# chengzhag/PanFusion

Hardware: AMD Instinct MI355X
Metric: DDIM denoise steps/sec, 512x1024 pano + 20x512^2 views (higher is better)
Workload: dtype fp16; 1 GPU; cfg2: 512x1024 pano + 20x512^2 views, CFG pair, SD-2-base UNet shapes; views=20, cfg_pair=True, hip_graphs=True, parallelism=single

## Files before the change

### include/panfusion_hip.h

```cpp
#ifndef PANFUSION_HIP_H
#define PANFUSION_HIP_H

#include <stddef.h>
#include <stdint.h>

#ifdef __cplusplus
extern "C" {
#endif

typedef enum { PF_OK = 0, PF_ERR_ARG = 1, PF_ERR_LAUNCH = 2, PF_ERR_UNSUPPORTED = 3 } pf_status;
typedef enum { PF_BF16 = 0, PF_F16 = 1, PF_F32 = 2, PF_U8 = 3, PF_F64 = 4 } pf_dtype;

int pf_version(void);
const char* pf_last_error_string(void);


pf_status pf_e2p_grid(const double* host_fov, const double* host_theta, const double* host_phi,
                      int ncam, int eh, int ew, int h, int w,
                      float* map_x, float* map_y, float* lonlat, void* stream);

pf_status pf_p2e_grid(const double* host_fov, const double* host_theta, const double* host_phi,
                      int ncam, int ph, int pw, int h, int w,
                      float* map_u, float* map_v, uint8_t* mask, void* stream);

// ... 164 lines not shown
    int h_out, w_out;
    int ksize;
    int stride;
    int pad;
    int upsample;
    const void* w;
    int n_out;
    const float* bias;
    const float* rowvec;
    int rowvec_ld;
    const void* residual;
    int res_ld;
    int res_dtype;
    void* out;
    int out_ld;
    int out_dtype;
    int dtype;
    int batch;
    long a_bstride, w_bstride, out_bstride, res_bstride;
    int epilogue;
    void* workspace;
    size_t workspace_bytes;
    float* gn_partial;
    int wrap_pad;
    int crop;
    int* tickets;
    int n_tickets;
    int split3;
    int subpixel;
    int gn_rows;
    int a_src_dtype;
    const float* a_scale;
    const float* a_shift;
} pf_conv_desc;

enum { PF_EPILOGUE_NONE = 0, PF_EPILOGUE_GEGLU = 1, PF_EPILOGUE_SPLIT = 2 };

size_t pf_conv_gemm_workspace_size(const pf_conv_desc* desc);
int pf_conv_gemm_gn_rows(const pf_conv_desc* desc);
int pf_conv_gemm_kernel_id(const pf_conv_desc* desc);
typedef struct {
    int kernel;
    int mrep, nrep;
    int block_rows;
    int waves;
    int ring_slots;
    int splits;
    int kb_per_split;
    int m_split;
    int tail_splits, tail_kb;
    int gn_rows;
    int n_tickets;
    size_t workspace_bytes;
} pf_conv_plan;
pf_status pf_conv_gemm_plan(const pf_conv_desc* desc, int want_moments, pf_conv_plan* out);
pf_status pf_debug_gemm_profile(void* device_buffer, long capacity_blocks);
pf_status pf_conv_gemm(const pf_conv_desc* desc, void* stream);

typedef struct {
    const void* a; int a_ld;
    const void* w;
    const float* bias;
    const float* residual; int res_ld;
    void* out; int out_ld;
    void* out_vt; int vt_ld; int rows_per_batch; long vt_bs;
    const float* ln_gamma; const float* ln_beta; float ln_eps; void* ln_out; int ln_ld;
// ... 179 lines not shown
```

### panfusion_amd/_lib.py

```python
import ctypes as C
import os

_HERE = os.path.dirname(os.path.abspath(__file__))
LIB_PATH = os.environ.get("PF_HIP_LIB") or os.path.join(_HERE, "libpanfusion_hip.so")

PF_OK = 0
PF_BF16, PF_F16, PF_F32, PF_U8, PF_F64 = 0, 1, 2, 3, 4

c_void_p, c_int, c_long, c_float, c_size_t = C.c_void_p, C.c_int, C.c_long, C.c_float, C.c_size_t
c_dp = C.POINTER(C.c_double)


class ConvDesc(C.Structure):
    _fields_ = [
        ("a0", c_void_p), ("a1", c_void_p), ("c0", c_int), ("c1", c_int),
        ("a0_ld", c_int), ("a1_ld", c_int),
        ("n_img", c_int), ("h_in", c_int), ("w_in", c_int), ("h_out", c_int), ("w_out", c_int),
        ("ksize", c_int), ("stride", c_int), ("pad", c_int), ("upsample", c_int),
        ("w", c_void_p), ("n_out", c_int),
        ("bias", c_void_p), ("rowvec", c_void_p), ("rowvec_ld", c_int),
        ("residual", c_void_p), ("res_ld", c_int), ("res_dtype", c_int),
        ("out", c_void_p), ("out_ld", c_int), ("out_dtype", c_int), ("dtype", c_int),
        ("batch", c_int),
        ("a_bstride", c_long), ("w_bstride", c_long), ("out_bstride", c_long), ("res_bstride", c_long),
        ("epilogue", c_int), ("workspace", c_void_p), ("workspace_bytes", c_size_t),
        ("gn_partial", c_void_p), ("wrap_pad", c_int), ("crop", c_int),
        ("tickets", c_void_p), ("n_tickets", c_int), ("split3", c_int), ("subpixel", c_int), ("gn_rows", c_int),
        ("a_src_dtype", c_int), ("a_scale", c_void_p), ("a_shift", c_void_p),
    ]


class ConvPlan(C.Structure):
    _fields_ = [
        ("kernel", c_int), ("mrep", c_int), ("nrep", c_int), ("block_rows", c_int), ("waves", c_int), ("ring_slots", c_int),
        ("splits", c_int), ("kb_per_split", c_int), ("m_split", c_int), ("tail_splits", c_int), ("tail_kb", c_int),
        ("gn_rows", c_int), ("n_tickets", c_int), ("workspace_bytes", c_size_t),
    ]


class AttnDesc(C.Structure):
    _fields_ = [
        ("q", c_void_p), ("k", c_void_p), ("vt", c_void_p), ("out", c_void_p),
        ("dtype", c_int), ("B", c_int), ("H", c_int), ("D", c_int), ("nq", c_int), ("nk", c_int),
        ("q_ld", c_int), ("k_ld", c_int), ("vt_ld", c_int), ("o_ld", c_int),
        ("q_bs", c_long), ("k_bs", c_long), ("vt_bs", c_long), ("o_bs", c_long),
        ("scale", c_float),
        ("bias", c_void_p), ("bias_ld", c_long), ("flags", c_void_p), ("flags_ld", c_int),
        ("lse", c_void_p),
        ("workspace", c_void_p), ("workspace_bytes", c_size_t),
    ]


class AttnPlan(C.Structure):
    _fields_ = [
        ("kernel", c_int), ("pipelined", c_int), ("occupancy", c_int), ("msum", c_int), ("block_queries", c_int), ("threads", c_int),
        ("splits", c_int), ("split_tiles", c_int), ("grid_x", C.c_uint), ("grid_y", C.c_uint), ("grid_z", C.c_uint),
        ("workspace_bytes", c_size_t),
    ]


class LinearWsDesc(C.Structure):
# ... 252 lines not shown
```

### panfusion_amd/csrc/pf_gemm.hip

```cpp
#include "pf_common.h"
#include "pf_gemm_params.h"
#include "pf_gemm_walk.h"
#include <stdlib.h>
#include <algorithm>
#include <atomic>
#include <type_traits>

namespace pf {


template <typename T> struct Mfma;
template <> struct Mfma<Bf16> {
    typedef __attribute__((ext_vector_type(8))) __bf16 frag;
    static __device__ __forceinline__ f32x4 run(frag a, frag b, f32x4 c) {
        return __builtin_amdgcn_mfma_f32_16x16x32_bf16(a, b, c, 0, 0, 0);
    }
    static __device__ __forceinline__ void acc_agpr(frag a, frag b, f32x4& c) {
        asm volatile("v_mfma_f32_16x16x32_bf16 %0, %1, %2, %0" : "+a"(c) : "v"(a), "v"(b));
    }
};
template <> struct Mfma<F16> {
    typedef __attribute__((ext_vector_type(8))) _Float16 frag;
    static __device__ __forceinline__ f32x4 run(frag a, frag b, f32x4 c) {
        return __builtin_amdgcn_mfma_f32_16x16x32_f16(a, b, c, 0, 0, 0);
// ... 1324 lines not shown
    GemmParams p;
    params_from_desc(d, p);
    const pf_conv_plan g = plan_conv_gemm(p, batch, d->workspace != nullptr, d->gn_partial != nullptr);
    PF_REQUIRE(!(a32 && d->a_scale && g.kernel == 1 && g.block_rows == 256 && g.nrep == 5),
               "pf_conv_gemm: a_scale / a_shift are not available on the 256 x 160 tile of the 8-wave kernel (this problem's plan): use the pair form");
    PF_REQUIRE(!(a32 && d->a_scale) || (d->h_out * d->w_out) % 2 == 0, "pf_conv_gemm: a_scale needs an even number of rows per image");
    if (d->gn_partial) {
        PF_REQUIRE(g.gn_rows > 0, "pf_conv_gemm: gn_partial given but this problem cannot emit GroupNorm moments (ask pf_conv_gemm_gn_rows first)");
        PF_REQUIRE(aligned16(d->gn_partial), "pf_conv_gemm: gn_partial must be 16-byte aligned");
        PF_REQUIRE(d->gn_rows == g.gn_rows, "pf_conv_gemm: gn_partial is sized for runs of gn_rows = %d rows, but this launch's plan writes runs of %d rows (ask pf_conv_gemm_plan again)",
                   d->gn_rows, g.gn_rows);
        p.gn_partial = d->gn_partial;
        p.gn_rows = g.gn_rows;
    }
    {
        const long npix = static_cast<long>(d->n_img) * d->h_in * d->w_in;
        const long a0b = a32 ? ((npix - 1) * p.a0_ld + p.c0 / 2) * 4 : ((npix - 1) * p.a0_ld + p.c0) * 2;
        const long a1b = !p.a1 ? 0 : a32 ? ((npix - 1) * p.a1_ld + p.c1 / 2) * 4 : ((npix - 1) * p.a1_ld + p.c1) * 2;
        const long wb = static_cast<long>(p.N) * p.K * 2;
        PF_REQUIRE(a0b < (1L << 31) && a1b < (1L << 31) && wb < (1L << 31),
                   "pf_conv_gemm: each operand must be smaller than 2 GiB (32-bit buffer offsets)");
        p.a0_bytes = static_cast<unsigned>(a0b); p.a1_bytes = static_cast<unsigned>(a1b); p.w_bytes = static_cast<unsigned>(wb);
    }
    p.partial = static_cast<float*>(d->workspace);
    if (d->tickets && g.kernel != 2 && gemm_tuning().splitk_inkernel && d->workspace_bytes < (1ULL << 32)) {
        PF_REQUIRE(d->n_tickets >= g.n_tickets && (reinterpret_cast<uintptr_t>(d->tickets) & 3) == 0,
                   "pf_conv_gemm: %d arrival counters needed, %d given", g.n_tickets, d->n_tickets);
        p.tickets = d->tickets;
    }
    PF_REQUIRE(g.workspace_bytes == 0 || (d->workspace_bytes >= g.workspace_bytes && aligned16(d->workspace)),
               "pf_conv_gemm: workspace of %zu bytes (16-byte aligned) needed, got %zu", g.workspace_bytes, d->workspace_bytes);
    hipStream_t st = as_stream(stream);
    p.splits = g.splits; p.kb_per_split = g.kb_per_split;
    if (g.m_split == 0) return launch_pass(g, p, d->dtype, batch, st);
    GemmParams p2 = p;
    p.M = g.m_split;
    p2.m_begin = g.m_split; p2.splits = g.tail_splits; p2.kb_per_split = g.tail_kb;
    const pf_status s1 = launch_pass(g, p, d->dtype, batch, st);
    return s1 != PF_OK ? s1 : launch_pass(g, p2, d->dtype, batch, st);
}

extern "C" pf_status pf_debug_gemm_profile(void* device_buffer, long capacity_blocks) {
    const ProfState* s = device_buffer ? new ProfState{static_cast<unsigned long long*>(device_buffer), capacity_blocks} : nullptr;
    g_prof_state.store(s, std::memory_order_release);
    return PF_OK;
}
```

### panfusion_amd/csrc/pf_gemm_params.h

```cpp
#pragma once
#include <atomic>
#include <cstdlib>

#include "pf_common.h"

namespace pf {

struct GemmParams {
    const unsigned short* a0; const unsigned short* a1;
    int c0, c1, a0_ld, a1_ld;
    int h_in, w_in, h_out, w_out;
    int ksize, stride, pad, up;
    int wrap, crop;
    const unsigned short* w;
    int M, N, K;
    int m_begin;
    int rows_per_img;
    const float* bias; const float* rowvec; int rowvec_ld;
    const void* residual; int res_ld; int res_f32;
    void* out; int out_ld; int out_f32; int geglu;
    int split_out;
    long a_bs, w_bs, out_bs, res_bs;
    int mtiles, ntiles;
    int splits, kb_per_split;
    float* partial;
    int* tickets;
    int batch;
    unsigned a0_bytes, a1_bytes, w_bytes;
    int adv_img, adv_y, adv_x;
    unsigned long long* prof;
    int s3;
    float* gn_partial;
    int gn_rows;
    int fastseg;
    int a32;
    const float* a_scale; const float* a_shift;
    int subpix;
};

__device__ __forceinline__ void seg_pack(int& img_pix, int& y_msk, int x, int h_in, int w_in) {
    const int img = img_pix, y = y_msk;
    unsigned m = 0;
#pragma unroll
    for (int k = 0; k < 3; ++k) {
        m |= (static_cast<unsigned>(y + k) < static_cast<unsigned>(h_in) ? 1u : 0u) << k;
        m |= (static_cast<unsigned>(x + k) < static_cast<unsigned>(w_in) ? 16u : 0u) << k;
    }
    img_pix = static_cast<int>((static_cast<unsigned>(img) * static_cast<unsigned>(h_in) + static_cast<unsigned>(y)) * static_cast<unsigned>(w_in) + static_cast<unsigned>(x));
    y_msk = static_cast<int>(m);
}

__device__ __forceinline__ long out_row(const GemmParams& p, long bz, int m) {
    if (!p.subpix) return m;
    const int q = m / p.w_out, x = m - q * p.w_out;
    return (2L * q + (bz >> 1)) * (2 * p.w_out) + 2 * x + (bz & 1);
}
__device__ __forceinline__ long gn_part(const GemmParams& p, long bz, int m) {
    if (!p.subpix) return m / p.gn_rows;
    const int img = m / p.rows_per_img, rem = m - img * p.rows_per_img, ppi = p.rows_per_img / p.gn_rows;
    return (static_cast<long>(img) * 4 + bz) * ppi + rem / p.gn_rows;
}

#ifdef PF_GEMM_TIMELINE
#define PF_TL(p, cond, slot) do { if ((cond) && (p).prof && threadIdx.x == 0) { const long b_ = blockIdx.x + static_cast<long>(gridDim.x) * (blockIdx.y + static_cast<long>(gridDim.y) * blockIdx.z); (p).prof[b_ * 32 + (slot)] = __builtin_amdgcn_s_memtime(); } } while (0)
#else
#define PF_TL(p, cond, slot) do { } while (0)
#endif
__device__ __forceinline__ void stamp(const GemmParams& p, int slot) {
    if (p.prof && threadIdx.x == 0) {
        const long b = blockIdx.x + static_cast<long>(gridDim.x) * (blockIdx.y + static_cast<long>(gridDim.y) * blockIdx.z);
// ... 34 lines not shown
        unsigned short* o = static_cast<unsigned short*>(p.out) + bz * p.out_bs + out_row(p, bz, m) * p.out_ld + n4;
        u16x4 hi, lo;
#pragma unroll
        for (int e = 0; e < 4; ++e) {
            hi[e] = from_f32<T>(v[e]);
            lo[e] = from_f32<T>(v[e] - to_f32<T>(hi[e]));
        }
        *reinterpret_cast<u16x4*>(o + (pair_off(n4) - n4)) = hi;
        *reinterpret_cast<u16x4*>(o + (pair_off(n4) - n4) + 32) = lo;
    } else if (p.out_f32) {
        float* o = static_cast<float*>(p.out) + bz * p.out_bs + out_row(p, bz, m) * p.out_ld + n4;
        *reinterpret_cast<float4*>(o) = float4{v[0], v[1], v[2], v[3]};
    } else {
        unsigned short* o = static_cast<unsigned short*>(p.out) + bz * p.out_bs + out_row(p, bz, m) * p.out_ld + n4;
        u16x4 w4;
#pragma unroll
        for (int e = 0; e < 4; ++e) w4[e] = from_f32<T>(v[e]);
        *reinterpret_cast<u16x4*>(o) = w4;
    }
}

__device__ __forceinline__ void slab_store(const GemmParams& p, long elem, const f32x4& v) {
    if (p.tickets) {
        typedef __attribute__((ext_vector_type(4))) unsigned int u32x4;
        const __amdgpu_buffer_rsrc_t rs = __builtin_amdgcn_make_buffer_rsrc(uniform_ptr(p.partial), 0, 0xFFFFFFFFu, 0x00020000);
        __builtin_amdgcn_raw_buffer_store_b128(__builtin_bit_cast(u32x4, v), rs, static_cast<int>(static_cast<unsigned>(elem * 4)), 0,  16);
    } else {
        *reinterpret_cast<float4*>(p.partial + elem) = float4{v[0], v[1], v[2], v[3]};
    }
}

pf_status launch_gemm32(const GemmParams& gp, int dtype, int batch, hipStream_t st);


struct GemmTuning {
    int deep_ring = env_int("PF_GEMM_DEEP_RING", 1);
    int deep_ring_max_blocks = env_int("PF_GEMM_DEEP_RING_MAX_BLOCKS", 256);
    int split_min_kb = env_int("PF_GEMM_SPLIT_MINKB", 12);
    int big_min_tiles = env_int("PF_GEMM8_MIN_TILES", 128);
    int big_fill_pct = env_int("PF_GEMM8_FILL", 30);
    int big_min_k = env_int("PF_GEMM8_MIN_K", 0);
    int big_waves = env_int("PF_GEMM8_WAVES", 8);
    int big_persist = env_int("PF_GEMM8_PERSIST", 256);
    int tail_split = env_int("PF_GEMM_TAIL_SPLIT", 1);
    int tail_first_pct = env_int("PF_GEMM8_TAIL_FIRST", 80);
    int tail_min_kb = env_int("PF_GEMM_TAIL_MINKB", 40);
    int bm128 = env_int("PF_GEMM_BM128", 2);
    int bm128_max_k = env_int("PF_GEMM_BM128_MAXK", 1280);
    int bm128_one_round = env_int("PF_GEMM_BM128_ONEROUND", 0);
    int gemm32_min_k = env_int("PF_GEMM32_MINK", 2560);
    int gemm32_k1 = env_int("PF_GEMM32_K1", 0);
    int gemm32_persist = env_int("PF_GEMM32_PERSIST", 256);
    int splitk_inkernel = env_int("PF_SPLITK_INKERNEL", 0);
    static int gemm32() { return env_int("PF_GEMM32", 0); }
    static int gn_epilogue_res() { return env_int("PF_GN_EPILOGUE_RES", 0); }
    static int conv_fastseg() { return env_int("PF_CONV_FASTSEG", 1); }
};
const GemmTuning& gemm_tuning();

void params_from_desc(const pf_conv_desc* d, GemmParams& p);
pf_conv_plan plan_conv_gemm(const GemmParams& p, int batch, bool allow_split, bool want_moments);

}
```

### panfusion_amd/csrc/pf_gemm_plan.hip

```cpp
#include "pf_gemm_params.h"

namespace pf {

const GemmTuning& gemm_tuning() {
    static const GemmTuning t;
    return t;
}

void params_from_desc(const pf_conv_desc* d, GemmParams& p) {
    const int c1 = d->a1 ? d->c1 : 0;
    const int Ctot = d->c0 + c1;
    p.a0 = static_cast<const unsigned short*>(d->a0);
    p.a1 = static_cast<const unsigned short*>(d->a1);
    p.c0 = d->c0; p.c1 = c1; p.a0_ld = d->a0_ld; p.a1_ld = d->a1 ? d->a1_ld : 0;
    p.h_in = d->h_in; p.w_in = d->w_in; p.h_out = d->h_out; p.w_out = d->w_out;
    p.ksize = d->ksize; p.stride = d->stride; p.pad = d->pad; p.up = d->upsample;
    p.wrap = d->wrap_pad; p.crop = d->crop;
    p.w = static_cast<const unsigned short*>(d->w);
    p.rows_per_img = d->h_out * d->w_out;
    p.M = d->n_img * p.rows_per_img; p.N = d->n_out; p.K = d->ksize * d->ksize * Ctot;
    p.bias = d->bias; p.rowvec = d->rowvec; p.rowvec_ld = d->rowvec_ld;
    p.residual = d->residual; p.res_ld = d->res_ld;
    p.res_f32 = d->residual != nullptr && d->res_dtype == PF_F32;
    p.out = d->out; p.out_ld = d->out_ld; p.out_f32 = d->out_dtype == PF_F32;
    p.geglu = d->epilogue == PF_EPILOGUE_GEGLU;
    p.split_out = d->epilogue == PF_EPILOGUE_SPLIT;
    p.a_bs = d->a_bstride; p.w_bs = d->w_bstride; p.out_bs = d->out_bstride; p.res_bs = d->res_bstride;
    p.mtiles = p.ntiles = 0;
    p.prof = nullptr;
    p.s3 = d->split3 != 0;
    p.batch = d->batch;
    p.gn_partial = nullptr; p.gn_rows = 0;
    p.m_begin = 0; p.splits = 1; p.kb_per_split = 0; p.partial = nullptr; p.tickets = nullptr;
    p.a0_bytes = p.a1_bytes = p.w_bytes = 0; p.adv_img = p.adv_y = p.adv_x = 0;
    p.a32 = d->a_src_dtype == PF_F32;
    p.a_scale = p.a32 ? d->a_scale : nullptr; p.a_shift = p.a32 ? d->a_shift : nullptr;
    if (p.a32) { p.c0 = 2 * d->c0; p.c1 = 2 * c1; p.K = 2 * Ctot; }
    p.subpix = 0;
    p.fastseg = (d->upsample == 0 || d->subpixel) && d->wrap_pad == 0 && GemmTuning::conv_fastseg() ? 1 : 0;
    if (d->subpixel) {
        p.subpix = 1; p.ksize = 2; p.up = 0; p.pad = 0;
        p.h_out = d->h_out / 2; p.w_out = d->w_out / 2;
        p.rows_per_img = p.h_out * p.w_out;
        p.M = d->n_img * p.rows_per_img; p.K = 4 * Ctot;
        p.crop = d->crop / 2;
        p.batch = 4; p.a_bs = 0; p.out_bs = 0; p.res_bs = 0; p.w_bs = static_cast<long>(p.N) * p.K;
    }
}


static pf_conv_plan plan_small(long M, int N, int K, int batch, bool allow_split, bool s3) {
    const GemmTuning& t = gemm_tuning();
    pf_conv_plan g{};
    g.kernel = 0;
    g.nrep = (N % 160 == 0) ? 5 : 4;
    const long ntiles = cdiv(N, 32 * g.nrep);
    const long tiles128 = cdiv(M, 128) * ntiles * batch;
    g.mrep = tiles128 < 512 ? 2 : 4;
    g.block_rows = 32 * g.mrep;
    const long tiles = cdiv(M, 32 * g.mrep) * ntiles * batch;
    const int nkb = K / 64;
    g.splits = 1;
    g.kb_per_split = nkb;
    if (t.deep_ring && !s3 && tiles <= 256) {
        long s = allow_split && N % 4 == 0 && nkb >= t.split_min_kb ? 256 / tiles : 1;
        if (s > nkb / 4) s = nkb / 4;
        if (s > 32) s = 32;
        if (s > 1) {
            g.kb_per_split = static_cast<int>(cdiv(nkb, s));
            g.splits = static_cast<int>(cdiv(nkb, g.kb_per_split));
        }
// ... 80 lines not shown
    return staged ? rows : 0;
}


static bool plan32(const GemmParams& p, int batch, bool allow_split, pf_conv_plan& g) {
    const GemmTuning& t = gemm_tuning();
    if (!GemmTuning::gemm32() || p.s3 || p.subpix || batch != 1 || p.N % 320 != 0 || p.K < t.gemm32_min_k || p.K % 64 != 0 || p.geglu)
        return false;
    if (p.ksize != 3 && !t.gemm32_k1) return false;
    const int nkb = p.K / 64;
    g = pf_conv_plan{};
    g.kernel = 2; g.mrep = 8; g.nrep = 10; g.block_rows = 256; g.splits = 1; g.kb_per_split = nkb;
    const long ntl = p.N / 320, mt = cdiv(p.M, 256), tiles = mt * ntl;
    const long full = tiles / 256 * 256, rest = tiles - full;
    if (rest == 0) return true;
    if (full == 0 || !allow_split || p.N % 4 != 0) return false;
    const long rows1 = full / ntl;
    long sp = (256 + rest / 2) / rest;
    if (sp > nkb / 8) sp = nkb / 8;
    if (sp < 2 || rest * sp > 256) return false;
    g.m_split = static_cast<int>(rows1 * 256);
    g.tail_kb = static_cast<int>(cdiv(nkb, sp));
    g.tail_splits = static_cast<int>(cdiv(nkb, g.tail_kb));
    return true;
}
static int gn_rows32(const GemmParams& p, const pf_conv_plan& g) {
    if (g.m_split > 0 || p.residual || p.split_out || p.geglu) return 0;
    if (p.rows_per_img % 64 != 0) return 0;
    const bool ok = p.out_f32 ? (p.out_ld & 3) == 0 : (p.out_ld & 7) == 0;
    return ok ? 64 : 0;
}


pf_conv_plan plan_conv_gemm(const GemmParams& p, int batch, bool allow_split, bool want_moments) {
    const GemmTuning& t = gemm_tuning();
    pf_conv_plan g{};
    if (plan32(p, batch, allow_split, g) && (!want_moments || gn_rows32(p, g) > 0)) {
        g.gn_rows = want_moments ? 64 : 0;
        g.waves = 8; g.ring_slots = 4;
    } else {
        g = plan_tiles(p.M, p.N, p.K, batch, allow_split, p.s3 != 0);
        g.gn_rows = want_moments ? gn_rows16(p, g, batch) : 0;
        if (p.a32 && g.kernel == 1) g.gn_rows = 0;
        if (g.kernel == 1) {
            if (takes_128_row_blocks(g, p.M, p.N, p.K, batch)) { g.block_rows = 128; g.waves = 4; g.ring_slots = 2; }
            else { g.waves = t.big_waves == 4 && !p.s3 ? 4 : 8; g.ring_slots = 3; }
        } else {
            const long blocks = cdiv(p.M, g.block_rows) * cdiv(p.N, 32 * g.nrep) * g.splits * batch;
            const int deep_max = t.deep_ring ? t.deep_ring_max_blocks : 0;
            g.waves = 4;
            g.ring_slots = g.gn_rows == 0 && !p.s3 && blocks <= deep_max && p.K / 64 / g.splits >= 3 ? 4 : 2;
        }
    }
    const long rows2 = p.M - g.m_split;
    if (g.m_split > 0) g.workspace_bytes = static_cast<size_t>(g.tail_splits) * rows2 * p.N * sizeof(float);
    else if (g.splits > 1) g.workspace_bytes = static_cast<size_t>(g.splits) * batch * p.M * p.N * sizeof(float);
    if (g.workspace_bytes && g.kernel != 2) g.n_tickets = static_cast<int>(cdiv(rows2, g.block_rows) * cdiv(p.N, 32 * g.nrep) * batch);
    return g;
}

}

using namespace pf;

extern "C" pf_status pf_conv_gemm_plan(const pf_conv_desc* d, int want_moments, pf_conv_plan* out) {
    PF_REQUIRE(d && out, "pf_conv_gemm_plan: null pointer");
    PF_REQUIRE(d->batch >= 1 && d->n_out >= 1 && d->n_img >= 1, "pf_conv_gemm_plan: batch, n_out and n_img must be >= 1");
    GemmParams p;
    params_from_desc(d, p);
// ... 21 lines not shown
```

### panfusion_amd/ops.py

```python
import ctypes as C
import os

import numpy as np
import torch

from . import _lib
from ._lib import (PF_BF16, PF_F16, PF_F32, PF_GN_FROM_PARTIALS, AttnBwdDesc, AttnBwdPlan, AttnDesc, AttnPlan, ConvDesc, ConvPlan, GnPlan,
                   LinearWsDesc, LwsPlan, check)

_DT = {torch.bfloat16: PF_BF16, torch.float16: PF_F16, torch.float32: PF_F32}

TRACE = None


class _PlanCache(__import__("threading").local):
    LIMIT = 4096

    def __init__(self):
        self.plans = {}


_PLANS = _PlanCache()
SPLITK_INKERNEL = os.environ.get("PF_SPLITK_INKERNEL") == "1"

# ... 517 lines not shown
    op_dtype = a32_dtype or a0.dtype
    c0 = c0 if c0 is not None else a0.shape[-1]
    c1 = (c1 if c1 is not None else a1.shape[-1]) if a1 is not None else 0
    if w_in is None:
        w_in = a0.numel() // (a0.shape[-1] * max(batch, 1)) if ksize == 1 else None
    hl, wl = h_in << upsample, (w_in + 2 * wrap_pad) << upsample
    h_out = (hl + 2 * pad + pad_hi - ksize) // stride + 1
    w_out = (wl + 2 * pad + pad_hi - ksize) // stride + 1 - 2 * crop
    M = n_img * h_out * w_out
    if out is not None:
        out_dtype = out.dtype
    if split_out:
        out_dtype = op_dtype
    out_dtype = out_dtype or (residual.dtype if residual is not None else op_dtype)
    n_store = n_out // 2 if geglu else (2 * n_out if split_out else n_out)
    if out is None and not want_plan:
        out = torch.empty((batch, M, n_store) if batch > 1 else (M, n_store), device=a0.device, dtype=out_dtype)
    a0_ld = a0_ld if a0_ld is not None else _ld(a0)
    a1_ld = (a1_ld if a1_ld is not None else _ld(a1)) if a1 is not None else 0
    rowvec_ld = _ld(rowvec) if rowvec is not None else 0
    res_ld = (res_ld if res_ld is not None else _ld(residual)) if residual is not None else 0
    res_dtype = dt(residual) if residual is not None else dt(op_dtype)
    out_ld = out_ld if out_ld is not None else (_ld(out) if out is not None else n_store)
    epilogue = 1 if geglu else (2 if split_out else 0)
    pkey = (c0, c1, a0_ld, a1_ld, n_img, h_in, w_in, h_out, w_out, ksize, stride, pad, upsample, n_out, batch, epilogue, wrap_pad,
            crop, dt(op_dtype), dt(out_dtype), residual is not None, res_dtype, res_ld, rowvec is not None, rowvec_ld, bias is not None,
            out_ld, a_bstride, w_bstride, out_bstride, res_bstride, bool(split3), bool(subpixel), PF_F32 if a32_dtype else 0, a_scale is not None)
    plans = _PLANS.plans
    plan = plans.get(pkey)
    if plan is None:
        d = _conv_desc(pkey)
        d.a0, d.a1, d.w, d.bias, d.rowvec, d.residual, d.out = _p(a0), _p(a1), _p(w), _p(bias), _p(rowvec), _p(residual), _p(out)
        d.a_scale, d.a_shift = _p(a_scale), _p(a_shift)
        if len(plans) >= _PLANS.LIMIT:
            plans.pop(next(iter(plans)))
        plan = plans[pkey] = [d, _conv_plan(d, 0), None]
    d = plan[0]
    if plan_only:
        return plan[1].kernel
    d.a0, d.a1, d.w, d.bias, d.rowvec, d.residual, d.out = _p(a0), _p(a1), _p(w), _p(bias), _p(rowvec), _p(residual), _p(out)
    d.a_scale, d.a_shift = _p(a_scale), _p(a_shift)
    d.gn_partial, d.gn_rows, d.tickets, d.n_tickets = None, 0, None, 0
    if want_plan:
        if gn_stats and GN_FROM_EPILOGUE and batch == 1 and plan[2] is None:
            plan[2] = _conv_plan(d, 1)
        return plan[2] if gn_stats and GN_FROM_EPILOGUE and batch == 1 and plan[2].gn_rows > 0 else plan[1]
    g, gn = plan[1], None
    if gn_stats and GN_FROM_EPILOGUE and batch == 1:
        if plan[2] is None:
            plan[2] = _conv_plan(d, 1)
        if plan[2].gn_rows > 0:
            g = plan[2]
            gn = (torch.empty(M // g.gn_rows, 2, n_out // 2, device=a0.device, dtype=torch.float32), g.gn_rows)
            d.gn_partial, d.gn_rows = _p(gn[0]), g.gn_rows
    nbytes = g.workspace_bytes if split_k else 0
    ws = torch.empty(nbytes, device=a0.device, dtype=torch.uint8) if nbytes else None
    d.workspace, d.workspace_bytes = _p(ws), nbytes
    if nbytes and SPLITK_INKERNEL:
        d.tickets, d.n_tickets = _ticket_slice(a0.device), _TICKET_SLICE
    if TRACE is None:
        check(_lib.lib().pf_conv_gemm(C.byref(d), _stream()), "pf_conv_gemm")
    else:
        _traced("k_conv_gemm", 2.0 * M * n_out * (algo_k or ksize * ksize * (c0 + c1)) * batch,
                lambda: check(_lib.lib().pf_conv_gemm(C.byref(d), _stream()), "pf_conv_gemm"),
                "M%d N%d K%d k%d s%d u%d b%d%s" % (M, n_out, ksize * ksize * (c0 + c1) * (2 if a32_dtype else 1), ksize, stride, upsample, batch, " g32" if plan[1].kernel == 2 else " subpixel" if subpixel else ""))
    if gn is not None:
# ... 539 lines not shown
```

Measured before the change: 17.27 steps/s.

## Add persistent 256x320-tile wide conv GEMM kernel for large-K 3x3 convolutions

Adds a new persistent implicit-GEMM kernel that uses 256x320 output tiles with 512 threads, double-buffered LDS DMA and interleaved MFMA/fragment reads. It serves 3x3 stride-1 convs with N a multiple of 320, K of at least 2560 and N up to 640. The row count is rounded so full waves of tiles go to the wide kernel, and leftover rows go to the existing big-tile kernel. Wider tiles raise operand reuse per loaded byte, at the cost of heavy register pressure, single-block occupancy and an extra launch for the tail.

```diff
diff --git a/include/panfusion_hip.h b/include/panfusion_hip.h
--- a/include/panfusion_hip.h
+++ b/include/panfusion_hip.h
@@ -220,6 +220,7 @@
     int a_src_dtype;
     const float* a_scale;
     const float* a_shift;
+    int wide;
 } pf_conv_desc;
 
 enum { PF_EPILOGUE_NONE = 0, PF_EPILOGUE_GEGLU = 1, PF_EPILOGUE_SPLIT = 2 };
diff --git a/panfusion_amd/_lib.py b/panfusion_amd/_lib.py
--- a/panfusion_amd/_lib.py
+++ b/panfusion_amd/_lib.py
@@ -26,7 +26,7 @@
         ("epilogue", c_int), ("workspace", c_void_p), ("workspace_bytes", c_size_t),
         ("gn_partial", c_void_p), ("wrap_pad", c_int), ("crop", c_int),
         ("tickets", c_void_p), ("n_tickets", c_int), ("split3", c_int), ("subpixel", c_int), ("gn_rows", c_int),
-        ("a_src_dtype", c_int), ("a_scale", c_void_p), ("a_shift", c_void_p),
+        ("a_src_dtype", c_int), ("a_scale", c_void_p), ("a_shift", c_void_p), ("wide", c_int),
     ]
 
 
diff --git a/panfusion_amd/csrc/pf_gemm.hip b/panfusion_amd/csrc/pf_gemm.hip
--- a/panfusion_amd/csrc/pf_gemm.hip
+++ b/panfusion_amd/csrc/pf_gemm.hip
@@ -1380,6 +1380,19 @@
                "pf_conv_gemm: workspace of %zu bytes (16-byte aligned) needed, got %zu", g.workspace_bytes, d->workspace_bytes);
     hipStream_t st = as_stream(stream);
     p.splits = g.splits; p.kb_per_split = g.kb_per_split;
+    if (g.kernel == 3) {
+        const int rows_wide = GemmTuning::gemm_wide() == 2 ? 0 : g.m_split > 0 ? g.m_split : p.M;
+        if (rows_wide > 0) {
+            GemmParams pw = p;
+            pw.M = rows_wide;
+            const pf_status s1 = launch_gemm_wide(pw, d->dtype, batch, st);
+            if (s1 != PF_OK || rows_wide == p.M) return s1;
+        }
+        pf_conv_plan tail{};
+        tail.kernel = 1; tail.mrep = 8; tail.nrep = 5; tail.block_rows = 256; tail.waves = 8; tail.ring_slots = 3; tail.splits = 1; tail.kb_per_split = g.kb_per_split;
+        p.m_begin = rows_wide;
+        return launch_pass(tail, p, d->dtype, batch, st);
+    }
     if (g.m_split == 0) return launch_pass(g, p, d->dtype, batch, st);
     GemmParams p2 = p;
     p.M = g.m_split;
diff --git a/panfusion_amd/csrc/pf_gemm_params.h b/panfusion_amd/csrc/pf_gemm_params.h
--- a/panfusion_amd/csrc/pf_gemm_params.h
+++ b/panfusion_amd/csrc/pf_gemm_params.h
@@ -36,6 +36,7 @@
     int a32;
     const float* a_scale; const float* a_shift;
     int subpix;
+    int wide;
 };
 
 __device__ __forceinline__ void seg_pack(int& img_pix, int& y_msk, int x, int h_in, int w_in) {
@@ -136,6 +137,9 @@
 
 pf_status launch_gemm32(const GemmParams& gp, int dtype, int batch, hipStream_t st);
 
+pf_status launch_gemm_wide(const GemmParams& gp, int dtype, int batch, hipStream_t st);
+bool gemm_wide_serves(const GemmParams& p, int batch);
+
 
 struct GemmTuning {
     int deep_ring = env_int("PF_GEMM_DEEP_RING", 1);
@@ -159,6 +163,10 @@
     static int gemm32() { return env_int("PF_GEMM32", 0); }
     static int gn_epilogue_res() { return env_int("PF_GN_EPILOGUE_RES", 0); }
     static int conv_fastseg() { return env_int("PF_CONV_FASTSEG", 1); }
+    static int gemm_wide() { return env_int("PF_GEMM_WIDE", 1); }
+    static int gemm_wide_min_k() { return env_int("PF_GEMM_WIDE_MINK", 2560); }
+    static int gemm_wide_max_n() { return env_int("PF_GEMM_WIDE_MAXN", 640); }
+    static int gemm_wide_round() { return env_int("PF_GEMM_WIDE_ROUND", 256); }
 };
 const GemmTuning& gemm_tuning();
 
diff --git a/panfusion_amd/csrc/pf_gemm_plan.hip b/panfusion_amd/csrc/pf_gemm_plan.hip
--- a/panfusion_amd/csrc/pf_gemm_plan.hip
+++ b/panfusion_amd/csrc/pf_gemm_plan.hip
@@ -37,6 +37,7 @@
     p.a_scale = p.a32 ? d->a_scale : nullptr; p.a_shift = p.a32 ? d->a_shift : nullptr;
     if (p.a32) { p.c0 = 2 * d->c0; p.c1 = 2 * c1; p.K = 2 * Ctot; }
     p.subpix = 0;
+    p.wide = d->wide;
     p.fastseg = (d->upsample == 0 || d->subpixel) && d->wrap_pad == 0 && GemmTuning::conv_fastseg() ? 1 : 0;
     if (d->subpixel) {
         p.subpix = 1; p.ksize = 2; p.up = 0; p.pad = 0;
@@ -183,9 +184,34 @@
 }
 
 
+bool gemm_wide_serves(const GemmParams& p, int batch) {
+    if (p.ksize != 3 || p.stride != 1 || p.up || p.wrap || p.crop || p.subpix || p.s3 || p.a32 || batch != 1 || p.geglu || p.split_out) return false;
+    if (p.N % 320 != 0 || p.K % 64 != 0) return false;
+    if (p.out_f32) return !p.rowvec && (p.out_ld & 3) == 0 && (!p.residual || (p.res_f32 && (p.res_ld & 3) == 0));
+    return !p.residual && (p.out_ld & 3) == 0 && (!p.rowvec || (p.rowvec_ld & 3) == 0);
+}
+
+static bool plan_wide(const GemmParams& p, int batch, bool want_moments, pf_conv_plan& g) {
+    if (!p.wide || GemmTuning::gemm_wide() == 0 || !gemm_wide_serves(p, batch)) return false;
+    if (p.K < GemmTuning::gemm_wide_min_k() || p.N > GemmTuning::gemm_wide_max_n()) return false;
+    const long round = GemmTuning::gemm_wide_round() > 0 ? GemmTuning::gemm_wide_round() : 1;
+    const long ntl = p.N / 320, mt = cdiv(p.M, 256);
+    const long rows1 = (mt * ntl / round * round) / ntl;
+    if (rows1 == 0) return false;
+    const pf_conv_plan tail = plan_big(5, p.K);
+    if (want_moments && (p.out_f32 || gn_rows16(p, tail, batch) != 64)) return false;
+    g = pf_conv_plan{};
+    g.kernel = 3; g.mrep = 8; g.nrep = 10; g.block_rows = 256; g.waves = 8; g.ring_slots = 2; g.splits = 1; g.kb_per_split = p.K / 64;
+    if (rows1 < mt) { g.m_split = static_cast<int>(rows1 * 256); g.tail_splits = 1; g.tail_kb = p.K / 64; }
+    g.gn_rows = want_moments ? 64 : 0;
+    return true;
+}
+
+
 pf_conv_plan plan_conv_gemm(const GemmParams& p, int batch, bool allow_split, bool want_moments) {
     const GemmTuning& t = gemm_tuning();
     pf_conv_plan g{};
+    if (plan_wide(p, batch, want_moments, g)) return g;
     if (plan32(p, batch, allow_split, g) && (!want_moments || gn_rows32(p, g) > 0)) {
         g.gn_rows = want_moments ? 64 : 0;
         g.waves = 8; g.ring_slots = 4;
diff --git a/panfusion_amd/csrc/pf_gemm_wide.hip b/panfusion_amd/csrc/pf_gemm_wide.hip
--- /dev/null
+++ b/panfusion_amd/csrc/pf_gemm_wide.hip
@@ -0,0 +1,393 @@
+#include "pf_common.h"
+#include "pf_gemm_params.h"
+#include "pf_gemm_walk.h"
+#include <stdlib.h>
+#include <algorithm>
+#include <type_traits>
+
+namespace pf {
+
+namespace gw {
+constexpr int BM = 256, BN = 320, BK = 64, SLOTS = 2, NT = 512;
+constexpr int STAGE = (BM + BN) * BK;
+constexpr int RPP = NT / 8;
+constexpr int APASS = BM / RPP, BPASS = BN / RPP, NPIECE = APASS + BPASS;
+constexpr int MI = 4, NJ = 10;
+constexpr int NG = 2 * NJ;
+static_assert(NPIECE == 9 && BN % RPP == 0, "the counted waits below");
+
+template <typename T> struct Mfma;
+template <> struct Mfma<Bf16> {
+    typedef __attribute__((ext_vector_type(8))) __bf16 frag;
+    static __device__ __forceinline__ f32x4 run(frag a, frag b, f32x4 c) { return __builtin_amdgcn_mfma_f32_16x16x32_bf16(a, b, c, 0, 0, 0); }
+};
+template <> struct Mfma<F16> {
+    typedef __attribute__((ext_vector_type(8))) _Float16 frag;
+    static __device__ __forceinline__ f32x4 run(frag a, frag b, f32x4 c) { return __builtin_amdgcn_mfma_f32_16x16x32_f16(a, b, c, 0, 0, 0); }
+};
+
+__device__ __forceinline__ int lds_off(int row, int chunk) {
+    return row * 64 + ((chunk ^ ((row >> 1) & 7)) << 3);
+}
+__device__ __forceinline__ float row16_allreduce(float v) {
+#define PF_ROR(n) __builtin_bit_cast(float, __builtin_amdgcn_update_dpp(0, __builtin_bit_cast(int, v), 0x120 + (n), 0xF, 0xF, false))
+    v += PF_ROR(8);
+    v += PF_ROR(4);
+    v += PF_ROR(2);
+    v += PF_ROR(1);
+#undef PF_ROR
+    return v;
+}
+
+
+typedef __attribute__((ext_vector_type(4))) unsigned int u32x4;
+typedef __attribute__((ext_vector_type(2))) unsigned int u32x2;
+__device__ __forceinline__ __amdgpu_buffer_rsrc_t whole_buffer(const void* ptr) {
+    return __builtin_amdgcn_make_buffer_rsrc(uniform_ptr(static_cast<const char*>(ptr)), 0, 0xFFFFFFFFu, 0x00020000);
+}
+
+template <bool RES>
+__device__ __forceinline__ void store_f32(const GemmParams& p, const f32x4 (&acc)[MI][NJ], int mw, int nw, int lane) {
+    const int cq = 4 * (lane >> 4), rl = lane & 15;
+    const __amdgpu_buffer_rsrc_t rs_res = whole_buffer(RES ? p.residual : p.out), rs_out = whole_buffer(p.out);
+    bool live[MI];
+    int roff[MI], ooff[MI];
+#pragma unroll
+    for (int i = 0; i < MI; ++i) {
+        const int m = mw + 16 * i + rl;
+        live[i] = m < p.M;
+        const int mc = min(m, p.M - 1);
+        roff[i] = (mc * p.res_ld + nw + cq) * 4;
+        ooff[i] = (mc * p.out_ld + nw + cq) * 4;
+    }
+    constexpr int JH = NJ / 2, NU = 2 * MI;
+    f32x4 r[2][JH];
+    auto request = [&](int u) __attribute__((always_inline)) {
+        if constexpr (RES) {
+            const int i = u >> 1, j0 = (u & 1) * JH;
+#pragma unroll
+            for (int jj = 0; jj < JH; ++jj) r[u & 1][jj] = __builtin_bit_cast(f32x4, __builtin_amdgcn_raw_buffer_load_b128(rs_res, roff[i] + 64 * (j0 + jj), 0, 0));
+        }
+    };
+    request(0);
+#pragma unroll
+    for (int u = 0; u < NU; ++u) {
+        if (u + 1 < NU) request(u + 1);
+        const int i = u >> 1, j0 = (u & 1) * JH;
+#pragma unroll
+        for (int jj = 0; jj < JH; ++jj) {
+            const int j = j0 + jj;
+            const float4 b = p.bias ? *reinterpret_cast<const float4*>(p.bias + nw + 16 * j + cq) : float4{0.f, 0.f, 0.f, 0.f};
+            f32x4 v = {acc[i][j][0] + b.x, acc[i][j][1] + b.y, acc[i][j][2] + b.z, acc[i][j][3] + b.w};
+            if constexpr (RES) { const f32x4 x = r[u & 1][jj]; v[0] += x[0]; v[1] += x[1]; v[2] += x[2]; v[3] += x[3]; }
+            if (live[i]) __builtin_amdgcn_raw_buffer_store_b128(__builtin_bit_cast(u32x4, v), rs_out, ooff[i] + 64 * j, 0, 0);
+        }
+    }
+}
+
+template <typename T, bool STATS, bool RV>
+__device__ __forceinline__ void store_16(const GemmParams& p, const f32x4 (&acc)[MI][NJ], int mw, int nw, int lane) {
+    const int cq = 4 * (lane >> 4), rl = lane & 15;
+    const __amdgpu_buffer_rsrc_t rs_out = whole_buffer(p.out), rs_rv = whole_buffer(RV ? static_cast<const void*>(p.rowvec) : p.out);
+    const int NP = p.N >> 1;
+    float* base = STATS ? p.gn_partial + static_cast<long>(mw / p.gn_rows) * 2 * NP : nullptr;
+    int rpi = p.rows_per_img;
+    asm volatile("" : "+s"(rpi));
+    const float* rv_wave = RV ? p.rowvec + static_cast<long>(mw / rpi) * p.rowvec_ld : nullptr;
+    bool live[MI];
+    int ooff[MI], rvoff[MI];
+#pragma unroll
+    for (int i = 0; i < MI; ++i) {
+        const int m = mw + 16 * i + rl;
+        live[i] = m < p.M;
+        const int mc = min(m, p.M - 1);
+        ooff[i] = (mc * p.out_ld + nw + cq) * 2;
+        rvoff[i] = RV ? ((mc / rpi) * p.rowvec_ld + nw + cq) * 4 : 0;
+    }
+#pragma unroll
+    for (int j = 0; j < NJ; ++j) {
+        const int n = nw + 16 * j + cq;
+        const float4 b = p.bias ? *reinterpret_cast<const float4*>(p.bias + n) : float4{0.f, 0.f, 0.f, 0.f};
+        f32x4 rv[MI];
+        if constexpr (RV) {
+#pragma unroll
+            for (int i = 0; i < MI; ++i) rv[i] = __builtin_bit_cast(f32x4, __builtin_amdgcn_raw_buffer_load_b128(rs_rv, rvoff[i] + 64 * j, 0, 0));
+        }
+        float4 c = b;
+        if constexpr (STATS && RV) {
+            const float4 x = *reinterpret_cast<const float4*>(rv_wave + n);
+            c.x += x.x; c.y += x.y; c.z += x.z; c.w += x.w;
+        }
+        float sm0 = 0.f, sm1 = 0.f, sq0 = 0.f, sq1 = 0.f;
+#pragma unroll
+        for (int i = 0; i < MI; ++i) {
+            float v[4] = {acc[i][j][0] + b.x, acc[i][j][1] + b.y, acc[i][j][2] + b.z, acc[i][j][3] + b.w};
+            if constexpr (RV) { v[0] += rv[i][0]; v[1] += rv[i][1]; v[2] += rv[i][2]; v[3] += rv[i][3]; }
+            u16x4 w4;
+#pragma unroll
+            for (int e = 0; e < 4; ++e) w4[e] = from_f32<T>(v[e]);
+            if (live[i]) __builtin_amdgcn_raw_buffer_store_b64(__builtin_bit_cast(u32x2, w4), rs_out, ooff[i] + 32 * j, 0, 0);
+            if constexpr (STATS) {
+                const float lf = live[i] ? 1.f : 0.f;
+                float x0 = acc[i][j][0] + c.x, x1 = acc[i][j][1] + c.y, x2 = acc[i][j][2] + c.z, x3 = acc[i][j][3] + c.w;
+                x0 *= lf; x1 *= lf; x2 *= lf; x3 *= lf;
+                sm0 += x0 + x1; sm1 += x2 + x3;
+                sq0 += x0 * x0 + x1 * x1; sq1 += x2 * x2 + x3 * x3;
+            }
+        }
+        if constexpr (STATS) {
+            const float s0 = row16_allreduce(sm0), s1 = row16_allreduce(sm1);
+            const float q0 = row16_allreduce(sq0), q1 = row16_allreduce(sq1);
+            if (rl == 0) {
+                *reinterpret_cast<float2*>(base + (n >> 1)) = float2{s0, s1};
+                *reinterpret_cast<float2*>(base + NP + (n >> 1)) = float2{q0, q1};
+            }
+        }
+    }
+}
+
+}
+
+template <typename T, bool STATS>
+__global__ __launch_bounds__(512, 1) void k_conv_gemm_wide(const GemmParams p_in) {
+    using namespace gw;
+    GemmParams p = p_in;
+    p.fastseg = 1; p.ksize = 3; p.stride = 1; p.up = 0; p.wrap = 0; p.crop = 0; p.subpix = 0; p.s3 = 0; p.a32 = 0; p.splits = 1;
+    extern __shared__ __attribute__((aligned(16))) unsigned short smem[];
+
+    const int ntile_total = p.mtiles * p.ntiles;
+    const unsigned short* a0 = p.a0;
+    const unsigned short* a1 = p.a1;
+    int m0 = 0, n0 = 0;
+
+    auto lane_id = []() __attribute__((always_inline)) {
+        int l;
+        asm volatile("v_mbcnt_lo_u32_b32 %0, -1, 0\n\tv_mbcnt_hi_u32_b32 %0, -1, %0" : "=&v"(l));
+        return l;
+    };
+    const int wave = __builtin_amdgcn_readfirstlane(static_cast<int>(threadIdx.x) >> 6);
+    const int lane = lane_id(), t = wave * 64 + lane;
+    const int wm = wave >> 1, wn = wave & 1;
+    const int chunk = t & 7, lrow = t >> 3;
+    const int lchunk8 = (chunk ^ ((lrow >> 1) & 7)) * 8;
+
+    const __amdgpu_buffer_rsrc_t rs_w = __builtin_amdgcn_make_buffer_rsrc(uniform_ptr(p.w), 0, __builtin_amdgcn_readfirstlane(p.w_bytes), 0x00020000);
+    unsigned w_off = 0;
+    const int w_pass = __builtin_amdgcn_readfirstlane(RPP * p.K * 2);
+
+    const int n_it = p.K / BK;
+    ConvWalk<APASS, BK, true, false> w;
+    w.init(p, 0);
+    auto set_tile = [&](int tile) __attribute__((always_inline)) {
+        const int tid_lin = xcd_tile(tile, ntile_total);
+        const int tile_m = static_cast<unsigned>(tid_lin) / static_cast<unsigned>(p.ntiles), tile_n = tid_lin - tile_m * p.ntiles;
+        m0 = p.m_begin + tile_m * BM;
+        n0 = tile_n * BN;
+        const int tt = wave * 64 + lane_id();
+        GemmParams q = p;
+        asm volatile("" : "+s"(q.rows_per_img), "+s"(q.w_out));
+        const int lrow = tt >> 3;
+        w.rows_by_advance(q, m0, lrow, RPP);
+        w_off = weight_row_offset(p, n0 + lrow, lchunk8);
+        w.start(p, 0, lchunk8);
+    };
+
+    int st_soff_a = 0, st_soff_w = 0;
+    auto stage_begin = [&]() __attribute__((always_inline)) { return w.stage_begin(p, a0, a1, st_soff_a, st_soff_w); };
+    auto stage_end = [&]() __attribute__((always_inline)) { w.stage_end(p, lchunk8); };
+    auto dma_piece = [&](const __amdgpu_buffer_rsrc_t& rs_a, int slot, int k) __attribute__((always_inline)) {
+        unsigned short* As = smem + slot * STAGE;
+        unsigned short* Bs = As + BM * BK;
+        if (k < APASS) lds_dma16(rs_a, As + (k * RPP + wave * 8) * BK, w.off[k], st_soff_a);
+        else lds_dma16(rs_w, Bs + ((k - APASS) * RPP + wave * 8) * BK, w_off, st_soff_w + (k - APASS) * w_pass);
+    };
+    auto dma_stage = [&](int slot) __attribute__((always_inline)) {
+        const __amdgpu_buffer_rsrc_t rs_a = stage_begin();
+#pragma unroll
+        for (int k = 0; k < NPIECE; ++k) dma_piece(rs_a, slot, k);
+        stage_end();
+    };
+
+    f32x4 acc[MI][NJ];
+    typedef typename Mfma<T>::frag frag;
+    const int frow = lane & 15, fchunk = lane >> 4;
+    int a_off[2], b_off[2];
+#pragma unroll
+    for (int h = 0; h < 2; ++h) {
+        a_off[h] = 2 * lds_off(wm * 16 * MI + frow, 4 * h + fchunk);
+        b_off[h] = 2 * (BM * BK + lds_off(wn * 16 * NJ + frow, 4 * h + fchunk));
+    }
+    const char* smem_b = reinterpret_cast<const char*>(smem);
+    frag fa[2][MI];
+    frag fb[4];
+    auto rd_a = [&](int slot, int h, int i) __attribute__((always_inline)) {
+        fa[h][i] = __builtin_bit_cast(frag, *reinterpret_cast<const u16x8*>(smem_b + (slot * STAGE * 2 + a_off[h] + i * 16 * BK * 2)));
+    };
+    auto rd_b = [&](int slot, int g) __attribute__((always_inline)) {
+        fb[g & 3] = __builtin_bit_cast(frag, *reinterpret_cast<const u16x8*>(smem_b + (slot * STAGE * 2 + b_off[g / NJ] + (g % NJ) * 16 * BK * 2)));
+    };
+    auto group = [&](int g, auto dma_tag, const __amdgpu_buffer_rsrc_t& rs_a, int slot, int piece0, int ra_slot = -1) __attribute__((always_inline)) {
+        constexpr bool DMA = decltype(dma_tag)::value;
+        const int h = g / NJ, j = g % NJ;
+#pragma unroll
+        for (int i = 0; i < MI; ++i) {
+            acc[i][j] = Mfma<T>::run(fb[g & 3], fa[h][i], acc[i][j]);
+            if (ra_slot >= 0 && i < 2) {
+                __builtin_amdgcn_sched_barrier(0);
+                rd_a(ra_slot, h ^ 1, i + 2);
+                __builtin_amdgcn_sched_barrier(0);
+            }
+            if constexpr (DMA) {
+                const int k = piece0 + (i >> 1);
+                if ((i & 1) && k < NPIECE) {
+                    __builtin_amdgcn_sched_barrier(0);
+                    dma_piece(rs_a, slot, k);
+                    __builtin_amdgcn_sched_barrier(0);
+                }
+            }
+        }
+    };
+    static_assert(NG % 4 == 0, "the weight-fragment ring closes over a stage");
+
+    const std::true_type YES;
+    const std::false_type NO;
+    int cur = 0;
+    auto head = [&](auto dma_tag, const __amdgpu_buffer_rsrc_t& rs_a, int dslot) __attribute__((always_inline)) {
+        constexpr bool DMA = decltype(dma_tag)::value;
+#pragma unroll
+        for (int g = 0; g < NG - 2; ++g) {
+            __builtin_amdgcn_sched_barrier(0);
+            rd_b(cur, g + 2);
+            if (g == 3) { rd_a(cur, 1, 0); rd_a(cur, 1, 1); }
+            __builtin_amdgcn_sched_barrier(0);
+            if (DMA && g < 3) group(g, YES, rs_a, dslot, 4 + 2 * g);
+            else group(g, NO, rs_a, dslot, 0, g == NJ - 1 ? cur : -1);
+        }
+        if constexpr (DMA) stage_end();
+    };
+    auto tail = [&](auto more_tag, auto dma_tag, __amdgpu_buffer_rsrc_t& rs_a) __attribute__((always_inline)) {
+        constexpr bool MORE = decltype(more_tag)::value, DMA = decltype(dma_tag)::value;
+        const int nxt = cur ^ 1;
+        __builtin_amdgcn_sched_barrier(0);
+        if constexpr (MORE) {
+            asm volatile("s_waitcnt vmcnt(0) lgkmcnt(0)" ::: "memory");
+            __builtin_amdgcn_s_barrier();
+            asm volatile("" ::: "memory");
+            if constexpr (DMA) rs_a = stage_begin();
+            rd_a(nxt, 0, 0);
+            rd_a(nxt, 0, 1);
+            rd_b(nxt, 0);
+            __builtin_amdgcn_sched_barrier(0);
+        }
+        if constexpr (DMA) group(NG - 2, YES, rs_a, cur, 0);
+        else group(NG - 2, NO, rs_a, cur, 0);
+        __builtin_amdgcn_sched_barrier(0);
+        if constexpr (MORE) {
+            rd_b(nxt, 1);
+            __builtin_amdgcn_sched_barrier(0);
+        }
+        if constexpr (DMA) group(NG - 1, YES, rs_a, cur, 2, nxt);
+        else group(NG - 1, NO, rs_a, cur, 0, MORE ? nxt : -1);
+    };
+    auto issue_prologue = [&]() __attribute__((always_inline)) {
+        dma_stage(0);
+        if (n_it > 1) dma_stage(1);
+    };
+
+    int tile = blockIdx.x;
+    set_tile(tile);
+    issue_prologue();
+    bool first = true;
+    for (;;) {
+#pragma unroll
+        for (int i = 0; i < MI; ++i)
+#pragma unroll
+            for (int j = 0; j < NJ; ++j) acc[i][j] = f32x4{0.f, 0.f, 0.f, 0.f};
+        if (first && n_it > 1) asm volatile("s_waitcnt vmcnt(9)" ::: "memory");
+        else asm volatile("s_waitcnt vmcnt(0)" ::: "memory");
+        __builtin_amdgcn_s_barrier();
+        asm volatile("" ::: "memory");
+        first = false;
+        cur = 0;
+#pragma unroll
+        for (int i = 0; i < MI; ++i) rd_a(cur, 0, i);
+        rd_b(cur, 0);
+        rd_b(cur, 1);
+        {
+            __amdgpu_buffer_rsrc_t rs_a = rs_w;
+            head(NO, rs_a, 0);
+            for (int it = 0; it + 2 < n_it; ++it) {
+                const int dslot = cur;
+                tail(YES, YES, rs_a);
+                cur ^= 1;
+                head(YES, rs_a, dslot);
+            }
+            if (n_it >= 2) {
+                tail(YES, NO, rs_a);
+                cur ^= 1;
+                head(NO, rs_a, 0);
+            }
+            tail(NO, NO, rs_a);
+        }
+
+        const int em0 = m0, en0 = n0;
+        const int next = tile + static_cast<int>(gridDim.x);
+        const bool has_next = next < ntile_total;
+        __builtin_amdgcn_sched_barrier(0);
+        {
+            const int mw = em0 + wm * 16 * MI, nw = en0 + wn * 16 * NJ;
+            const int e_lane = lane_id();
+            if (mw < p.M) {
+                if (p.out_f32) {
+                    if (p.residual) store_f32<true>(p, acc, mw, nw, e_lane);
+                    else store_f32<false>(p, acc, mw, nw, e_lane);
+                } else {
+                    if (p.rowvec) store_16<T, STATS, true>(p, acc, mw, nw, e_lane);
+                    else store_16<T, STATS, false>(p, acc, mw, nw, e_lane);
+                }
+            }
+        }
+        if (!has_next) break;
+        __builtin_amdgcn_sched_barrier(0);
+        __syncthreads();
+        set_tile(next);
+        issue_prologue();
+        tile = next;
+    }
+}
+
+
+template <typename T, bool STATS>
+static pf_status launch_wide_s(const GemmParams& gp, hipStream_t st) {
+    using namespace gw;
+    GemmParams p = gp;
+    p.mtiles = static_cast<int>(cdiv(p.M - p.m_begin, BM));
+    p.ntiles = p.N / BN;
+    {
+        const int rem = RPP % p.rows_per_img;
+        p.adv_img = RPP / p.rows_per_img;
+        p.adv_y = rem / p.w_out;
+        p.adv_x = rem % p.w_out;
+    }
+    p.prof = nullptr;
+    const size_t smem = static_cast<size_t>(SLOTS) * STAGE * sizeof(unsigned short);
+    static std::atomic<unsigned long long> lds_set{0};
+    const pf_status s = allow_dynamic_lds(reinterpret_cast<const void*>(k_conv_gemm_wide<T, STATS>), smem, lds_set, "pf_conv_gemm (wide)");
+    if (s != PF_OK) return s;
+    const int grid = std::max(1, std::min(p.mtiles * p.ntiles, GemmTuning::gemm_wide_round()));
+    hipLaunchKernelGGL((k_conv_gemm_wide<T, STATS>), dim3(grid), dim3(NT), smem, st, p);
+    PF_CHECK_LAUNCH("pf_conv_gemm (wide)");
+    return PF_OK;
+}
+
+pf_status launch_gemm_wide(const GemmParams& gp, int dtype, int batch, hipStream_t st) {
+    PF_REQUIRE(gemm_wide_serves(gp, batch), "pf_conv_gemm (wide): 3x3 stride-1 convolutions with N a multiple of 320 only -- no split K, sub-pixel phases, "
+               "upsampling, circular wrap, crop, split precision, batch, GEGLU / pair output; 16-bit rows (+ bias, row vector) or fp32 rows (+ bias, fp32 residual)");
+    PF_REQUIRE(gp.splits == 1 && gp.M > gp.m_begin, "pf_conv_gemm (wide): no split K, at least one row");
+    PF_REQUIRE(!gp.gn_partial || (!gp.out_f32 && gp.gn_rows == 16 * gw::MI && gp.rows_per_img % gp.gn_rows == 0),
+               "pf_conv_gemm (wide): GroupNorm moments come with 16-bit rows, in runs of 64 rows that images are whole multiples of");
+    PF_DISPATCH_16(dtype, "pf_conv_gemm", return gp.gn_partial ? launch_wide_s<T, true>(gp, st) : launch_wide_s<T, false>(gp, st));
+    return PF_OK;
+}
+
+}
diff --git a/panfusion_amd/ops.py b/panfusion_amd/ops.py
--- a/panfusion_amd/ops.py
+++ b/panfusion_amd/ops.py
@@ -573,6 +573,8 @@
         d = _conv_desc(pkey)
         d.a0, d.a1, d.w, d.bias, d.rowvec, d.residual, d.out = _p(a0), _p(a1), _p(w), _p(bias), _p(rowvec), _p(residual), _p(out)
         d.a_scale, d.a_shift = _p(a_scale), _p(a_shift)
+        d.wide = int(ksize == 3 and stride == 1 and not (upsample or wrap_pad or crop or split3 or subpixel or geglu or split_out)
+                     and batch == 1 and n_out % 320 == 0)
         if len(plans) >= _PLANS.LIMIT:
             plans.pop(next(iter(plans)))
         plan = plans[pkey] = [d, _conv_plan(d, 0), None]
```

After: 17.40 steps/s, median of 6. About the same (+0.8%).
